# sjtuytc/UnboundedNeRFPytorch

Hardware: NVIDIA B200
Metric: ray-samples/sec (fwd+bwd train step) 8192x512 (higher is better)
Workload: dtype f32

## Files before the change

### include/ubnerf_b200.h

```cpp
#ifndef UBNERF_B200_H_
#define UBNERF_B200_H_

#include <stdint.h>

#ifdef __cplusplus
extern "C" {
#endif
#if defined(__GNUC__)
#pragma GCC visibility push(default)
#endif

#define UBN_ABI_VERSION 3

int ubn_abi_version(void);
const char* ubn_last_error_string(void);
int64_t ubn_launch_count(void);
void ubn_reset_launch_count(void);


int ubn_infer_t_minmax(const float* rays_o, const float* rays_d, const float* xyz_min, const float* xyz_max,
                       float near, float far, int64_t n_rays, float* t_min, float* t_max, void* stream);

int ubn_infer_n_samples(const float* rays_d, const float* t_min, const float* t_max, float stepdist,
                        int64_t n_rays, int64_t* n_samples, void* stream);
// ... 164 lines not shown
                          const UbnGridDesc* k0_desc, const UbnMarchCfg* cfg, int64_t n_rays,
                          const uint8_t* flags, const int64_t* offsets, const float* grad_feat,
                          float* grad_k0, void* stream);

int ubn_march_density_bwd(const float* rays_o, const float* rays_d, const float* t_table,
                          const UbnGridDesc* density_desc, const UbnMarchCfg* cfg, int64_t n_rays,
                          const float* density, const float* alpha, const float* weight, const float* T,
                          const uint8_t* flags, const float* alphainv_last, const int64_t* offsets,
                          const float* g_weight, const float* g_alpha, const float* g_density,
                          const float* g_last, float* grad_density_grid, void* stream);

int ubn_rgbnet_fwd(const float* feat, const float* view_bias, const int64_t* ray_id, const float* W1k, const float* W2,
                   const float* b2, const float* W3, const float* b3, int64_t n_pts, float* rgb, float* h1_save,
                   float* h2_save, void* stream);
int ubn_rgbnet_fwd_tc(const float* feat, const float* view_bias, const int64_t* ray_id, const float* W1k, const float* W2,
                      const float* b2, const float* W3, const float* b3, int64_t n_pts, float* rgb, float* h1_save,
                      float* h2_save, uint32_t* h1_mask, int single_pass, void* stream);
int ubn_rgbnet_bwd(const float* feat, const int64_t* ray_id, const float* W1k, const float* W2, const float* W3,
                   const float* rgb, const float* h1_save, const float* h2_save, const float* grad_rgb, int64_t n_pts,
                   float* grad_feat, float* grad_view_bias, float* grad_W1k, float* grad_W2, float* grad_b2,
                   float* grad_W3, float* grad_b3, void* stream);

int ubn_rgbnet_bwd_tc_data(const float* W2, const float* W3, const float* rgb, const float* h1_save, const float* h2_save,
                           const float* grad_rgb, int64_t n_pts, float* dz1_out, float* grad_W2, void* stream);
int ubn_rgbnet_bwd_small(const float* feat, const int64_t* ray_id, const float* W1k, const float* W3, const float* rgb,
                         const float* h2_save, const float* grad_rgb, const float* dz1, int64_t n_pts, float* grad_feat,
                         float* grad_view_bias, float* grad_W1k, float* grad_b2, float* grad_W3, float* grad_b3, void* stream);

int ubn_rgbnet_bwd_tc_fused(const float* feat, const int64_t* ray_id, const float* W1k, const float* W2, const float* W3,
                            const float* rgb, const float* h1_save, const float* h2_save, const float* grad_rgb, int64_t n_pts,
                            float* grad_feat, float* grad_view_bias, float* grad_W1k, float* grad_W2, float* grad_b2,
                            float* grad_W3, float* grad_b3, uint32_t* h2_mask_scratch, const uint32_t* h1_mask, int single_pass,
                            void* stream);

#if defined(__GNUC__)
#pragma GCC visibility pop
#endif
#ifdef __cplusplus
}
#endif
#endif
```

### unboundednerfpytorch_b200/_cabi.py

```python
import ctypes
import os

import torch

_HERE = os.path.dirname(os.path.abspath(__file__))
LIB_PATH = os.path.join(_HERE, 'libubnerf_b200.so')

c_i64 = ctypes.c_int64
c_i32 = ctypes.c_int32
c_int = ctypes.c_int
c_f = ctypes.c_float
c_p = ctypes.c_void_p


class UbnGridDesc(ctypes.Structure):
    _fields_ = [('P', c_i32), ('C', c_i32), ('X', c_i32), ('Y', c_i32), ('Z', c_i32), ('num_freqs', c_i32),
                ('stride_p', c_i64), ('stride_c', c_i64), ('stride_v', c_i64),
                ('xyz_min', c_f * 3), ('xyz_max', c_f * 3)]


class UbnMarchCfg(ctypes.Structure):
    _fields_ = [('scene_center', c_f * 3), ('scene_radius', c_f * 3),
                ('contract_B', c_f), ('contract_A', c_f),
                ('contracted_norm', c_i32), ('n_samples', c_i32),
                ('act_shift', c_f), ('interval', c_f), ('fast_color_thres', c_f),
                ('use_cumdist', c_i32), ('cumdist_thres', c_f),
                ('use_maskcache', c_i32), ('mask_sz', c_i32 * 3), ('mask_scale', c_f * 3), ('mask_shift', c_f * 3)]


ABI_VERSION = 3
FLAG_QUERIED, FLAG_LISTED, FLAG_SCANNED, FLAG_KEEP, FLAG_INNER = 1, 2, 4, 8, 16

_SIGNATURES = {
    'ubn_abi_version': [],
    'ubn_last_error_string': [],
    'ubn_launch_count': [],
    'ubn_reset_launch_count': [],
    'ubn_infer_t_minmax': [c_p, c_p, c_p, c_p, c_f, c_f, c_i64, c_p, c_p, c_p],
    'ubn_infer_n_samples': [c_p, c_p, c_p, c_f, c_i64, c_p, c_p],
    'ubn_infer_ray_start_dir': [c_p, c_p, c_p, c_i64, c_p, c_p, c_p],
    'ubn_sample_pts_count': [c_p, c_p, c_p, c_p, c_f, c_f, c_f, c_i64, c_p, c_p, c_p, c_p, c_p, c_p],
    'ubn_sample_pts_emit': [c_p, c_p, c_p, c_p, c_p, c_p, c_f, c_i64, c_i64, c_p, c_p, c_p, c_p, c_p],
    'ubn_sample_ndc_pts_on_rays': [c_p, c_p, c_p, c_p, c_i64, c_i64, c_p, c_p, c_p],
    'ubn_sample_bg_pts_on_rays': [c_p, c_p, c_p, c_f, c_i64, c_i64, c_p, c_p],
    'ubn_maskcache_lookup': [c_p, c_p, c_p, c_p, c_i64, c_i64, c_i64, c_i64, c_p, c_p],
    'ubn_raw2alpha': [c_p, c_f, c_f, c_p, c_i64, c_p, c_p, c_p],
    'ubn_raw2alpha_backward': [c_p, c_p, c_f, c_p, c_i64, c_p, c_p],
    'ubn_alpha2weight': [c_p, c_p, c_i64, c_i64, c_p, c_p, c_p, c_p, c_p, c_p],
    'ubn_alpha2weight_backward': [c_p, c_p, c_p, c_p, c_p, c_p, c_i64, c_i64, c_p, c_p, c_p, c_p],
    'ubn_segment_sum': [c_p, c_i64, c_p, c_i64, c_i64, c_p, c_p, c_p, c_p],
    'ubn_rgbnet_fwd': [c_p] * 8 + [c_i64] + [c_p] * 4,
    'ubn_rgbnet_fwd_tc': [c_p] * 8 + [c_i64] + [c_p] * 4 + [c_int, c_p],
    'ubn_rgbnet_bwd_tc_data': [c_p] * 6 + [c_i64] + [c_p] * 3,
    'ubn_rgbnet_bwd_small': [c_p] * 8 + [c_i64] + [c_p] * 7,
    'ubn_rgbnet_bwd': [c_p] * 9 + [c_i64] + [c_p] * 8,
    'ubn_rgbnet_bwd_tc_fused': [c_p] * 9 + [c_i64] + [c_p] * 9 + [c_int, c_p],
    'ubn_total_variation_add_grad': [c_p, c_p, c_f, c_f, c_f, c_i64, c_i64, c_i64, c_i64, c_i64, c_int, c_p],
    'ubn_adam_upd': [c_p, c_p, c_p, c_p, c_p, c_i64, c_int, c_f, c_f, c_f, c_f, c_int, c_p],
    'ubn_tv_adam_fused': [c_p, c_p, c_p, c_p, c_f, c_f, c_f, c_i64, c_i64, c_i64, c_i64, c_i64, c_int, c_int,
                          c_f, c_f, c_f, c_f, c_int, c_int, c_p],
    'ubn_tv_adam_pingpong': [c_p, c_p, c_p, c_p, c_p, c_f, c_f, c_f, c_i64, c_i64, c_i64, c_i64, c_i64, c_int, c_int,
                             c_f, c_f, c_f, c_f, c_int, c_int, c_p],
    'ubn_tv_adam_peer': [c_p, c_p, c_p, c_int, c_p, c_p, c_f, c_f, c_f, c_i64, c_i64, c_i64, c_i64, c_i64, c_int, c_i64, c_i64,
                         c_int, c_f, c_f, c_f, c_f, c_int, c_p],
    'ubn_lattice_alpha': [c_p, ctypes.POINTER(UbnGridDesc), c_p, c_p, c_i64, c_i64, c_i64, c_f, c_f, c_p, c_p],
    'ubn_maxpool3_gt_and': [c_p, c_i64, c_i64, c_i64, c_f, c_p, c_p],
    'ubn_resample_grid': [c_p, ctypes.POINTER(UbnGridDesc), c_p, ctypes.POINTER(UbnGridDesc), c_p],
    'ubn_view_scatter_ones': [c_p, c_p, c_i64, c_i64, c_f, c_f, c_f, ctypes.POINTER(UbnGridDesc), c_p, c_p],
    'ubn_count_gt': [c_p, c_f, c_i64, c_p, c_p],
    'ubn_maskout_near_cam': [c_p, c_i64, c_i64, c_i64, c_i64, c_p, c_i64, c_f, c_f, c_p],
    'ubn_cumdist_thres': [c_p, c_f, c_i64, c_i64, c_p, c_p],
    'ubn_get_rays_of_a_view': [c_int, c_int, c_p, c_p, c_int, c_int, c_int, c_int, c_int, c_int, c_p, c_p, c_p, c_p, c_p],
    'ubn_gather_rays': [c_p, c_p, c_int, c_p, c_i64, c_i64, c_p, c_p],
    'ubn_composite_fwd': [c_p, c_p, c_p, c_i64, c_i64, c_p, c_p, c_p, c_p],
    'ubn_composite_bwd': [c_p, c_p, c_p, c_p, c_i64, c_p, c_p, c_p],
    'ubn_distortion_loss': [c_p, c_p, c_p, c_i64, c_i64, c_f, c_p, c_p, c_p, c_p, c_p, c_i64, c_p],
    'ubn_render_loss': [c_p] * 7 + [c_i64, c_i64] + [c_f] * 6 + [c_p] * 6 + [c_i64, c_p],
    'ubn_grid_sample_fwd': [c_p, ctypes.POINTER(UbnGridDesc), c_p, c_i64, c_p, c_p],
    'ubn_grid_sample_bwd': [c_p, ctypes.POINTER(UbnGridDesc), c_p, c_i64, c_p, c_p],
    'ubn_march_density_fwd': [c_p, c_p, c_p, c_p, ctypes.POINTER(UbnGridDesc), c_p, ctypes.POINTER(UbnMarchCfg), c_i64,
                              c_p, c_p, c_p, c_p, c_p, c_p, c_p, c_p],
    'ubn_exclusive_scan_i32': [c_p, c_i64, c_p, c_p, c_p],
    'ubn_march_feature_fwd': [c_p, c_p, c_p, c_p, ctypes.POINTER(UbnGridDesc), ctypes.POINTER(UbnMarchCfg), c_i64,
                              c_p, c_p, c_p, c_p, c_p, c_p, c_p, c_p, c_p, c_p, c_p, c_p, c_p, c_p],
    'ubn_march_feature_fwd_tma': [c_p, c_p, c_p, c_p, ctypes.POINTER(UbnGridDesc), ctypes.POINTER(UbnMarchCfg), c_i64,
                                  c_p, c_p, c_p, c_p, c_p, c_p, c_p, c_p, c_p, c_p, c_p, c_p, c_p, c_p, c_p],
    'ubn_set_feature_kernel': [c_int],
    'ubn_get_feature_kernel': [],
    'ubn_set_density_scatter': [c_int],
# ... 99 lines not shown
```

### unboundednerfpytorch_b200/csrc/shade_tc.cu

```cuda
#include <algorithm>

#include "common.cuh"

namespace ubn {

namespace tc {

constexpr int kRows = 128;
constexpr int kHidden = 128;
constexpr int kFeat = 12;
constexpr int kK1 = 16;
constexpr uint32_t kPanelBytes = kRows * 16;
constexpr uint32_t kLBO = kPanelBytes;
constexpr uint32_t kSBO = 128;

constexpr uint32_t oW2hi = 0;
constexpr uint32_t oW2lo = oW2hi + (kHidden / 4) * kPanelBytes;
constexpr uint32_t oW1hi = oW2lo + (kHidden / 4) * kPanelBytes;
constexpr uint32_t oW1lo = oW1hi + (kK1 / 4) * kPanelBytes;
constexpr uint32_t oA1hi = oW1lo + (kK1 / 4) * kPanelBytes;
constexpr uint32_t oA1lo = oA1hi + (kK1 / 4) * kPanelBytes;
constexpr uint32_t oW3 = oA1lo + (kK1 / 4) * kPanelBytes;
constexpr uint32_t oB2 = oW3 + 3 * kHidden * 4;
constexpr uint32_t oBar = oB2 + kHidden * 4;
// ... 237 lines not shown
        for (int e = 0; e < 4; ++e) {
          const uint32_t hb = tf32_hi_bits(hs[e]);
          hi[q * 4 + e] = hb;
          lo[q * 4 + e] = __float_as_uint(hs[e] - __uint_as_float(hb));
        }
      }
      tmem_st32(tmem + lane_base + cA2hi + c * 32, hi);
      if (kThreePass) tmem_st32(tmem + lane_base + cA2lo + c * 32, lo);
      tmem_st_wait();
      tc_fence_before();
      __syncthreads();
      if (warp == 0 && elect_one()) {
        tc_fence_after();
#pragma unroll
        for (int hh = 0; hh < kHalves; ++hh) {
#pragma unroll
          for (int k4 = 0; k4 < 4; ++k4) {
            const int ks = (hh * kChunksPerHalf + cc) * 4 + k4;
            mma_ts(tmem + cD2, tmem + cA2hi + ks * 8, dW2hi + ks * kStep, (cc > 0 || hh > 0 || k4 > 0) ? 1u : 0u);
            if (kThreePass) {
              mma_ts(tmem + cD2, tmem + cA2lo + ks * 8, dW2hi + ks * kStep, 1);
              mma_ts(tmem + cD2, tmem + cA2hi + ks * 8, dW2lo + ks * kStep, 1);
            }
          }
        }
        if (cc == kChunksPerHalf - 1) mma_commit(bar_addr);
      }
      if (kSave) {
        if (kPanel && h1_mask) {
          uint32_t w = 0;
#pragma unroll
          for (int e = 31; e >= 0; --e) w = __funnelshift_l(__float_as_uint(__fsub_rn(0.f, v[e])), w, 1);
          h1_mask[tile * 512 + c * 128 + rtid] = live ? w : 0u;
          float* stg = reinterpret_cast<float*>(smem + oStg + warp * kStgBytesPerWarp);
          const int ln = tid & 31;
#pragma unroll
          for (int q = 0; q < 8; ++q)
            *reinterpret_cast<float4*>(stg + ln * kStgStride + q * 4) = make_float4(v[q * 4], v[q * 4 + 1], v[q * 4 + 2], v[q * 4 + 3]);
          __syncwarp();
          float* dstT = h1_out + tile * (kRows * kHidden) + (int64_t)(8 * (warp & 3)) * (kHidden * 4) + (c * 32 + ln) * 4;
#pragma unroll
          for (int q = 0; q < 8; ++q)
            *reinterpret_cast<float4*>(dstT + q * (kHidden * 4)) =
                make_float4(stg[(4 * q) * kStgStride + ln], stg[(4 * q + 1) * kStgStride + ln], stg[(4 * q + 2) * kStgStride + ln],
                            stg[(4 * q + 3) * kStgStride + ln]);
          __syncwarp();
        } else if (kPanel) {
          float4* dst = reinterpret_cast<float4*>(h1_out + tile * (kRows * kHidden) + (int64_t)(c * 8) * (kRows * 4) + rtid * 4);
#pragma unroll
          for (int q = 0; q < 8; ++q) dst[q * kRows] = make_float4(v[q * 4], v[q * 4 + 1], v[q * 4 + 2], v[q * 4 + 3]);
        } else {
          warp_store_chunk(reinterpret_cast<float*>(smem + oStg + warp * kStgBytesPerWarp), v,
                           h1_out + (tile * kRows + (warp & 3) * 32) * kHidden, c * 32, n_pts - (tile * kRows + (warp & 3) * 32), tid & 31);
        }
      }
    }
    mbar_wait(bar_addr, phase);
    phase ^= 1;
    tc_fence_after();
    float p0 = 0.f, p1 = 0.f, p2 = 0.f;
#pragma unroll 1
    for (int cc = 0; cc < kChunksPerHalf; ++cc) {
      const int c = half * kChunksPerHalf + cc;
      float v[32];
      tmem_ld32(tmem + lane_base + cD2 + c * 32, v);
#pragma unroll
      for (int q = 0; q < 8; ++q) {
        const float4 bb = *reinterpret_cast<const float4*>(sB2 + c * 32 + q * 4);
        const float4 wa = *reinterpret_cast<const float4*>(sW3 + c * 32 + q * 4);
        const float4 wb = *reinterpret_cast<const float4*>(sW3 + kHidden + c * 32 + q * 4);
        const float4 wc = *reinterpret_cast<const float4*>(sW3 + 2 * kHidden + c * 32 + q * 4);
        const float h0 = fmaxf(v[q * 4] + bb.x, 0.f), h1v = fmaxf(v[q * 4 + 1] + bb.y, 0.f);
        const float h2v = fmaxf(v[q * 4 + 2] + bb.z, 0.f), h3 = fmaxf(v[q * 4 + 3] + bb.w, 0.f);
        v[q * 4] = h0; v[q * 4 + 1] = h1v; v[q * 4 + 2] = h2v; v[q * 4 + 3] = h3;
        p0 = fmaf(h3, wa.w, fmaf(h2v, wa.z, fmaf(h1v, wa.y, fmaf(h0, wa.x, p0))));
        p1 = fmaf(h3, wb.w, fmaf(h2v, wb.z, fmaf(h1v, wb.y, fmaf(h0, wb.x, p1))));
        p2 = fmaf(h3, wc.w, fmaf(h2v, wc.z, fmaf(h1v, wc.y, fmaf(h0, wc.x, p2))));
      }
      if (kSave) {
// ... 1303 lines not shown
      for (int ks = 0; ks < (int)(kK / 8); ++ks) {
        mma_ss(tmem + cAcc, dAhi + ks * kStepK, dBhi + ks * kStepK, (!fresh || ks > 0) ? 1u : 0u);
        if (kThree) {
          mma_ss(tmem + cAcc, dAlo + ks * kStepK, dBhi + ks * kStepK, 1);
          mma_ss(tmem + cAcc, dAhi + ks * kStepK, dBlo + ks * kStepK, 1);
        }
      }
      mma_commit(bar_addr);
    }
    pending = true;
    prefetch(rd + 1);
  }
  if (pending) {
    mbar_wait(bar_addr, phase);
    tc_fence_after();
    fold(n_folded == 0);
#pragma unroll 1
    for (int c = 0; c < 2; ++c) {
      float v[32];
      tmem_ld32(my_tmem + cSum + c * 32, v);
      float* dst = gW2 + ((warp & 3) * 32 + lane) * kHidden + (warp >> 2) * 64 + c * 32;
#pragma unroll
      for (int e = 0; e < 32; ++e) atomicAdd(dst + e, v[e]);
    }
  }
#pragma unroll
  for (int i = 0; i < 4; ++i) atomicAdd(sB2 + 32 * i + lane, accb[i]);
  tc_fence_before();
  __syncthreads();
  if (tid < kHidden && gb2) atomicAdd(gb2 + tid, sB2[tid]);
  if (warp == 0) asm volatile("tcgen05.dealloc.cta_group::1.sync.aligned.b32 %0, 256;" ::"r"(tmem) : "memory");
}

}
}

using namespace ubn;

extern "C" int ubn_rgbnet_fwd_tc(const float* feat, const float* view_bias, const int64_t* ray_id, const float* W1k,
                                 const float* W2, const float* b2, const float* W3, const float* b3, int64_t n_pts,
                                 float* rgb, float* h1_save, float* h2_save, uint32_t* h1_mask, int single_pass, void* stream) {
  if (n_pts <= 0) return 0;
  const bool save = h1_save != nullptr && h2_save != nullptr;
  const int64_t n_tiles = (n_pts + tc::kRows - 1) / tc::kRows;
  const unsigned grid = (unsigned)std::min<int64_t>(kNumSMs, n_tiles);
  cudaStream_t st = as_stream(stream);
#define UBN_TC_LAUNCH_H(SAVE, THREE, H, P)                                                                                \
  do {                                                                                                                  \
    cudaError_t e = cudaFuncSetAttribute(tc::k_shade_fwd_tc<SAVE, THREE, H, P>, cudaFuncAttributeMaxDynamicSharedMemorySize, \
                                         (int)tc::kSmemBytes);                                                          \
    if (e != cudaSuccess) return finish(e);                                                                             \
    tc::k_shade_fwd_tc<SAVE, THREE, H, P><<<grid, tc::kRows * H, tc::kSmemBytes, st>>>(feat, view_bias, ray_id, W1k, W2, b2, W3, \
                                                                                        b3, n_pts, rgb, h1_save, h2_save,    \
                                                                                        (SAVE && P) ? h1_mask : nullptr);    \
  } while (0)
#define UBN_TC_LAUNCH(SAVE, THREE, P)                                \
  do {                                                               \
    if (four_warps) UBN_TC_LAUNCH_H(SAVE, THREE, 1, P);              \
    else UBN_TC_LAUNCH_H(SAVE, THREE, 2, P);                         \
  } while (0)
  const bool four_warps = (single_pass & 2) != 0, panel = (single_pass & 4) != 0;
  single_pass &= 1;
  if (save && panel) {
    if (single_pass) UBN_TC_LAUNCH(true, false, true); else UBN_TC_LAUNCH(true, true, true);
  } else if (save) {
    if (single_pass) UBN_TC_LAUNCH(true, false, false); else UBN_TC_LAUNCH(true, true, false);
  } else {
    if (single_pass) UBN_TC_LAUNCH(false, false, false); else UBN_TC_LAUNCH(false, true, false);
  }
#undef UBN_TC_LAUNCH
#undef UBN_TC_LAUNCH_H
  UBN_LAUNCH_CHECK();
  return 0;
}


extern "C" int ubn_rgbnet_bwd_tc_data(const float* W2, const float* W3, const float* rgb, const float* h1_save,
                                      const float* h2_save, const float* grad_rgb, int64_t n_pts, float* dz1_out,
                                      float* grad_W2, void* stream) {
  if (n_pts <= 0) return 0;
  cudaStream_t st = as_stream(stream);
  {
    const int64_t n_tiles = (n_pts + tc::kRows - 1) / tc::kRows;
    const unsigned grid = (unsigned)std::min<int64_t>(kNumSMs, n_tiles);
    cudaError_t e = cudaFuncSetAttribute(tc::k_shade_bwd_tc<false>, cudaFuncAttributeMaxDynamicSharedMemorySize,
                                         (int)tc::bw::kSmemBytesB);
    if (e != cudaSuccess) return finish(e);
    tc::k_shade_bwd_tc<false><<<grid, tc::kRows, tc::bw::kSmemBytesB, st>>>(W2, W3, rgb, h1_save, h2_save, grad_rgb, n_pts,
                                                                            dz1_out, grad_W2);
    UBN_LAUNCH_CHECK();
  }
  {
    const int64_t n_rounds = (n_pts + tc::dw::kK - 1) / tc::dw::kK;
    const unsigned grid = (unsigned)std::min<int64_t>((int64_t)kNumSMs * tc::dw::kCtasPerSM, n_rounds);
    cudaError_t e = cudaFuncSetAttribute(tc::k_shade_dw2_tc<true, false>, cudaFuncAttributeMaxDynamicSharedMemorySize,
                                         (int)tc::dw::kSmemBytesD);
    if (e != cudaSuccess) return finish(e);
    tc::k_shade_dw2_tc<true, false><<<grid, tc::dw::kThreadsDW, tc::dw::kSmemBytesD, st>>>(W3, rgb, h1_save, h2_save, grad_rgb, n_pts,
                                                                                   grad_W2);
    UBN_LAUNCH_CHECK();
  }
  return 0;
}


extern "C" int ubn_rgbnet_bwd_tc_fused(const float* feat, const int64_t* ray_id, const float* W1k, const float* W2, const float* W3,
                                       const float* rgb, const float* h1_save, const float* h2_save, const float* grad_rgb,
                                       int64_t n_pts, float* grad_feat, float* grad_view_bias, float* grad_W1k, float* grad_W2,
                                       float* grad_b2, float* grad_W3, float* grad_b3, uint32_t* h2_mask_scratch,
                                       const uint32_t* h1_mask, int single_pass, void* stream) {
  if (n_pts <= 0) return 0;
  cudaStream_t st = as_stream(stream);
  {
    const int64_t n_tiles = (n_pts + tc::kRows - 1) / tc::kRows;
    const unsigned grid = (unsigned)std::min<int64_t>(kNumSMs, n_tiles);
#define UBN_BF(T)                                                                                                              \
    do {                                                                                                                       \
      cudaError_t e = cudaFuncSetAttribute(tc::k_shade_bwd_fused<T>, cudaFuncAttributeMaxDynamicSharedMemorySize,              \
                                           (int)tc::bf::kSmemBytesF);                                                          \
      if (e != cudaSuccess) return finish(e);                                                                                  \
      tc::k_shade_bwd_fused<T><<<grid, tc::kRows, tc::bf::kSmemBytesF, st>>>(feat, ray_id, W1k, W2, W3, rgb, h1_save, h2_save, grad_rgb, \
                                                                             n_pts, grad_feat, grad_view_bias, grad_W1k, grad_b2,       \
                                                                             grad_W3, grad_b3);                                         \
    } while (0)
#define UBN_BFW(T, P, M1)                                                                                                      \
    do {                                                                                                                       \
      cudaError_t e = cudaFuncSetAttribute(tc::k_shade_bwd_fused_ws<T, P, M1>, cudaFuncAttributeMaxDynamicSharedMemorySize,    \
                                           (int)tc::bf2::kSmemBytesF2);                                                        \
      if (e != cudaSuccess) return finish(e);                                                                                  \
      tc::k_shade_bwd_fused_ws<T, P, M1><<<grid, 2 * tc::kRows, tc::bf2::kSmemBytesF2, st>>>(                                  \
          feat, ray_id, W1k, W2, W3, rgb, h1_save, h2_save, grad_rgb, n_pts, grad_feat, grad_view_bias, grad_W1k, grad_b2, grad_W3,   \
          grad_b3, (P) ? h2_mask_scratch : nullptr, h1_mask);                                                                  \
    } while (0)
    const bool one_pass = (single_pass & 1) != 0, plain = (single_pass & 2) != 0, panel = (single_pass & 4) != 0;
    if (plain && panel) return finish(cudaErrorInvalidValue);
    if (plain)      { if (one_pass) UBN_BF(false); else UBN_BF(true); }
    else if (panel && h1_mask && h2_mask_scratch) { if (one_pass) UBN_BFW(false, true, true); else UBN_BFW(true, true, true); }
    else if (panel)            { if (one_pass) UBN_BFW(false, true, false); else UBN_BFW(true, true, false); }
    else                       { if (one_pass) UBN_BFW(false, false, false); else UBN_BFW(true, false, false); }
#undef UBN_BFW
#undef UBN_BF
    UBN_LAUNCH_CHECK();
  }
  {
    const int64_t n_rounds = (n_pts + tc::dw::kK - 1) / tc::dw::kK;
    const unsigned grid = (unsigned)std::min<int64_t>((int64_t)kNumSMs * tc::dw::kCtasPerSM, n_rounds);
#define UBN_DW(T, P)                                                                                                           \
    do {                                                                                                                       \
      cudaError_t e = cudaFuncSetAttribute(tc::k_shade_dw2_tc<T, P>, cudaFuncAttributeMaxDynamicSharedMemorySize,              \
                                           (int)tc::dw::kSmemBytesD);                                                          \
      if (e != cudaSuccess) return finish(e);                                                                                  \
      tc::k_shade_dw2_tc<T, P><<<grid, tc::dw::kThreadsDW, tc::dw::kSmemBytesD, st>>>(W3, rgb, h1_save, h2_save, grad_rgb, n_pts, grad_W2); \
    } while (0)
#define UBN_DWM(T)                                                                                                             \
    do {                                                                                                                       \
      cudaError_t e = cudaFuncSetAttribute(tc::k_shade_dw2_mask_tc<T>, cudaFuncAttributeMaxDynamicSharedMemorySize,            \
                                           (int)tc::dw::kSmemBytesD);                                                          \
      if (e != cudaSuccess) return finish(e);                                                                                  \
      tc::k_shade_dw2_mask_tc<T><<<grid, tc::dw::kThreadsDW, tc::dw::kSmemBytesD, st>>>(W3, rgb, h1_save, h2_mask_scratch, grad_rgb, n_pts, \
                                                                                      grad_W2, grad_b2);                       \
    } while (0)
    const bool from_masks = (single_pass & 4) && !(single_pass & 2) && h2_mask_scratch != nullptr && h1_mask != nullptr;
    if (from_masks)           { if (single_pass & 1) UBN_DWM(false); else UBN_DWM(true); }
    else if (single_pass & 4) { if (single_pass & 1) UBN_DW(false, true); else UBN_DW(true, true); }
    else                      { if (single_pass & 1) UBN_DW(false, false); else UBN_DW(true, false); }
#undef UBN_DWM
#undef UBN_DW
    UBN_LAUNCH_CHECK();
  }
  return 0;
}
```

### unboundednerfpytorch_b200/shade.py

```python
import torch

import os

from . import _cabi, ops
from ._cabi import c_i64, c_int, check, ptr, stream_of

MODE = os.environ.get('UBN_RGBNET_MODE', 'tc3')
BWD_MODE = os.environ.get('UBN_RGBNET_BWD_MODE', 'fused')
USE_MASKS = os.environ.get('UBN_RGBNET_MASKS', '1') == '1'


class _ShadeFn(torch.autograd.Function):
    @staticmethod
    def forward(ctx, feat, vb, ray_id, W1k, W2, b2, W3, b3, need_grad):
        feat, vb, ray_id = feat.contiguous(), vb.contiguous(), ray_id.contiguous()
        W1k, W2, b2, W3, b3 = (t.contiguous() for t in (W1k, W2, b2, W3, b3))
        M = feat.shape[0]
        dev = feat.device
        rgb = torch.empty(M, 3, dtype=torch.float32, device=dev)
        need_grad = bool(need_grad) and any(ctx.needs_input_grad)
        panel = need_grad and MODE in ('tc3', 'tc1', 'tc3w4') and BWD_MODE == 'fused'
        rows = -(-M // 128) * 128 if panel else M
        h1 = torch.empty(rows, 128, dtype=torch.float32, device=dev) if need_grad else None
        h2 = torch.empty(rows, 128, dtype=torch.float32, device=dev) if need_grad else None
        m1 = torch.empty(rows * 4, dtype=torch.int32, device=dev) if (panel and USE_MASKS) else None
        with ops._Guard(feat) as lib:
            with _cabi.timed('rgbnet_fwd'):
                if MODE in ('tc3', 'tc1', 'tc3w4'):
                    check(lib.ubn_rgbnet_fwd_tc(ptr(feat), ptr(vb), ptr(ray_id), ptr(W1k), ptr(W2), ptr(b2), ptr(W3), ptr(b3),
                                                c_i64(M), ptr(rgb), ptr(h1), ptr(h2), ptr(m1),
                                                c_int((1 if MODE == 'tc1' else 0) | (2 if MODE == 'tc3w4' else 0) | (4 if panel else 0)),
                                                stream_of(feat)))
                else:
                    check(lib.ubn_rgbnet_fwd(ptr(feat), ptr(vb), ptr(ray_id), ptr(W1k), ptr(W2), ptr(b2), ptr(W3), ptr(b3),
                                             c_i64(M), ptr(rgb), ptr(h1), ptr(h2), stream_of(feat)))
        if need_grad:
            ctx.save_for_backward(feat, ray_id, W1k, W2, W3, rgb, h1, h2)
            ctx.m1 = m1
            ctx.n_rays = vb.shape[0]
            ctx.panel = panel
            ctx.bwd_mode = BWD_MODE
        return rgb

    @staticmethod
    @torch.autograd.function.once_differentiable
    def backward(ctx, g_rgb):
        feat, ray_id, W1k, W2, W3, rgb, h1, h2 = ctx.saved_tensors
        dev = feat.device
        M = feat.shape[0]
        g_rgb = g_rgb.contiguous()
        g_feat = torch.empty_like(feat)
        z = lambda *s: torch.zeros(*s, dtype=torch.float32, device=dev)
        g_vb, gW1k, gW2, gb2, gW3, gb3 = z(ctx.n_rays, 128), z(128, 12), z(128, 128), z(128), z(3, 128), z(3)
        with ops._Guard(feat) as lib:
            bwd_mode = ctx.bwd_mode
            if bwd_mode in ('fused', 'fused4'):
                masks = torch.empty(-(-M // 128) * 512, dtype=torch.int32, device=dev) if (ctx.panel and ctx.m1 is not None) else None
                with _cabi.timed('rgbnet_bwd'):
                    check(lib.ubn_rgbnet_bwd_tc_fused(ptr(feat), ptr(ray_id), ptr(W1k), ptr(W2), ptr(W3), ptr(rgb), ptr(h1), ptr(h2),
                                                      ptr(g_rgb), c_i64(M), ptr(g_feat), ptr(g_vb), ptr(gW1k), ptr(gW2), ptr(gb2),
                                                      ptr(gW3), ptr(gb3), ptr(masks), ptr(ctx.m1 if bwd_mode == 'fused' else None), c_int((1 if MODE == 'tc1' else 0) | (2 if bwd_mode == 'fused4' else 0) | (4 if ctx.panel else 0)),
                                                      stream_of(feat)))
                return g_feat, g_vb, None, gW1k, gW2, gb2, gW3, gb3, None
            if bwd_mode == 'tc3':
                dz1 = torch.empty(M, 128, dtype=torch.float32, device=dev)
                with _cabi.timed('rgbnet_bwd'):
                    check(lib.ubn_rgbnet_bwd_tc_data(ptr(W2), ptr(W3), ptr(rgb), ptr(h1), ptr(h2), ptr(g_rgb), c_i64(M),
                                                     ptr(dz1), ptr(gW2), stream_of(feat)))
                with _cabi.timed('rgbnet_bwd_small'):
                    check(lib.ubn_rgbnet_bwd_small(ptr(feat), ptr(ray_id), ptr(W1k), ptr(W3), ptr(rgb), ptr(h2), ptr(g_rgb),
                                                   ptr(dz1), c_i64(M), ptr(g_feat), ptr(g_vb), ptr(gW1k), ptr(gb2), ptr(gW3),
                                                   ptr(gb3), stream_of(feat)))
                return g_feat, g_vb, None, gW1k, gW2, gb2, gW3, gb3, None
            with _cabi.timed('rgbnet_bwd'):
                check(lib.ubn_rgbnet_bwd(ptr(feat), ptr(ray_id), ptr(W1k), ptr(W2), ptr(W3), ptr(rgb), ptr(h1), ptr(h2),
                                         ptr(g_rgb), c_i64(M), ptr(g_feat), ptr(g_vb), ptr(gW1k), ptr(gW2), ptr(gb2),
                                         ptr(gW3), ptr(gb3), stream_of(feat)))
        return g_feat, g_vb, None, gW1k, gW2, gb2, gW3, gb3, None


def supported(rgbnet, k0_dim):
    try:
        l1, l2, l3 = rgbnet[0], rgbnet[2][0], rgbnet[3]
    except Exception:
        return False
    return (len(rgbnet) == 4 and k0_dim == 12 and l1.weight.shape[0] == 128 and tuple(l2.weight.shape) == (128, 128)
            and tuple(l3.weight.shape) == (3, 128) and l1.weight.is_cuda and l1.weight.dtype == torch.float32)


def shade(rgbnet, k0, view_emb, ray_id):
    l1, l2, l3 = rgbnet[0], rgbnet[2][0], rgbnet[3]
# ... 4 lines not shown
```

Before: 337.1 million.

## Recompute h1 activations in backward instead of saving them in forward

The forward pass no longer writes the full h1 activation tensor when masks are in use. A new backward kernel recomputes h1 on tensor cores from feat, W1k and the saved view bias, then accumulates grad_W2 and grad_b2 from it. This removes an M×128 float write in forward and the matching read in backward, at the cost of extra layer-1 MMA work and per-row gathers of the view bias in backward.

Result: slower. 325.4 million, median of 6 (-3.4%).

```diff
diff --git a/include/ubnerf_b200.h b/include/ubnerf_b200.h
--- a/include/ubnerf_b200.h
+++ b/include/ubnerf_b200.h
@@ -220,6 +220,11 @@
                             float* grad_feat, float* grad_view_bias, float* grad_W1k, float* grad_W2, float* grad_b2,
                             float* grad_W3, float* grad_b3, uint32_t* h2_mask_scratch, const uint32_t* h1_mask, int single_pass,
                             void* stream);
+int ubn_rgbnet_bwd_tc_recompute(const float* feat, const float* view_bias, const int64_t* ray_id, const float* W1k,
+                                const float* W2, const float* W3, const float* rgb, const float* h2_save, const float* grad_rgb,
+                                int64_t n_pts, float* grad_feat, float* grad_view_bias, float* grad_W1k, float* grad_W2,
+                                float* grad_b2, float* grad_W3, float* grad_b3, uint32_t* h2_mask_scratch,
+                                const uint32_t* h1_mask, int single_pass, void* stream);
 
 #if defined(__GNUC__)
 #pragma GCC visibility pop
diff --git a/unboundednerfpytorch_b200/_cabi.py b/unboundednerfpytorch_b200/_cabi.py
--- a/unboundednerfpytorch_b200/_cabi.py
+++ b/unboundednerfpytorch_b200/_cabi.py
@@ -55,6 +55,7 @@
     'ubn_rgbnet_bwd_small': [c_p] * 8 + [c_i64] + [c_p] * 7,
     'ubn_rgbnet_bwd': [c_p] * 9 + [c_i64] + [c_p] * 8,
     'ubn_rgbnet_bwd_tc_fused': [c_p] * 9 + [c_i64] + [c_p] * 9 + [c_int, c_p],
+    'ubn_rgbnet_bwd_tc_recompute': [c_p] * 9 + [c_i64] + [c_p] * 9 + [c_int, c_p],
     'ubn_total_variation_add_grad': [c_p, c_p, c_f, c_f, c_f, c_i64, c_i64, c_i64, c_i64, c_i64, c_int, c_p],
     'ubn_adam_upd': [c_p, c_p, c_p, c_p, c_p, c_i64, c_int, c_f, c_f, c_f, c_f, c_int, c_p],
     'ubn_tv_adam_fused': [c_p, c_p, c_p, c_p, c_f, c_f, c_f, c_i64, c_i64, c_i64, c_i64, c_i64, c_int, c_int,
diff --git a/unboundednerfpytorch_b200/csrc/shade_tc.cu b/unboundednerfpytorch_b200/csrc/shade_tc.cu
--- a/unboundednerfpytorch_b200/csrc/shade_tc.cu
+++ b/unboundednerfpytorch_b200/csrc/shade_tc.cu
@@ -293,19 +293,21 @@
 #pragma unroll
           for (int e = 31; e >= 0; --e) w = __funnelshift_l(__float_as_uint(__fsub_rn(0.f, v[e])), w, 1);
           h1_mask[tile * 512 + c * 128 + rtid] = live ? w : 0u;
-          float* stg = reinterpret_cast<float*>(smem + oStg + warp * kStgBytesPerWarp);
-          const int ln = tid & 31;
-#pragma unroll
-          for (int q = 0; q < 8; ++q)
-            *reinterpret_cast<float4*>(stg + ln * kStgStride + q * 4) = make_float4(v[q * 4], v[q * 4 + 1], v[q * 4 + 2], v[q * 4 + 3]);
-          __syncwarp();
-          float* dstT = h1_out + tile * (kRows * kHidden) + (int64_t)(8 * (warp & 3)) * (kHidden * 4) + (c * 32 + ln) * 4;
-#pragma unroll
-          for (int q = 0; q < 8; ++q)
-            *reinterpret_cast<float4*>(dstT + q * (kHidden * 4)) =
-                make_float4(stg[(4 * q) * kStgStride + ln], stg[(4 * q + 1) * kStgStride + ln], stg[(4 * q + 2) * kStgStride + ln],
-                            stg[(4 * q + 3) * kStgStride + ln]);
-          __syncwarp();
+          if (h1_out != nullptr) {
+            float* stg = reinterpret_cast<float*>(smem + oStg + warp * kStgBytesPerWarp);
+            const int ln = tid & 31;
+#pragma unroll
+            for (int q = 0; q < 8; ++q)
+              *reinterpret_cast<float4*>(stg + ln * kStgStride + q * 4) = make_float4(v[q * 4], v[q * 4 + 1], v[q * 4 + 2], v[q * 4 + 3]);
+            __syncwarp();
+            float* dstT = h1_out + tile * (kRows * kHidden) + (int64_t)(8 * (warp & 3)) * (kHidden * 4) + (c * 32 + ln) * 4;
+#pragma unroll
+            for (int q = 0; q < 8; ++q)
+              *reinterpret_cast<float4*>(dstT + q * (kHidden * 4)) =
+                  make_float4(stg[(4 * q) * kStgStride + ln], stg[(4 * q + 1) * kStgStride + ln], stg[(4 * q + 2) * kStgStride + ln],
+                              stg[(4 * q + 3) * kStgStride + ln]);
+            __syncwarp();
+          }
         } else if (kPanel) {
           float4* dst = reinterpret_cast<float4*>(h1_out + tile * (kRows * kHidden) + (int64_t)(c * 8) * (kRows * 4) + rtid * 4);
 #pragma unroll
@@ -1675,6 +1677,315 @@
   if (warp == 0) asm volatile("tcgen05.dealloc.cta_group::1.sync.aligned.b32 %0, 256;" ::"r"(tmem) : "memory");
 }
 
+namespace dr {
+constexpr int kThreadsDR = 256;
+constexpr uint32_t kOpBytes = (dw::kK / 4) * kPanelBytes;
+constexpr uint32_t oV1hi = 0;
+constexpr uint32_t oV1lo = oV1hi + (kK1 / 4) * kPanelBytes;
+constexpr uint32_t oXhi = oV1lo + (kK1 / 4) * kPanelBytes;
+constexpr uint32_t oXlo = oXhi + (kK1 / 4) * kPanelBytes;
+constexpr uint32_t oZ = oXlo + (kK1 / 4) * kPanelBytes;
+constexpr uint32_t oRayR = oZ + 4 * kOpBytes;
+constexpr uint32_t oB2R = oRayR + kRows * 8;
+constexpr uint32_t oBarR = oB2R + kHidden * 4;
+constexpr uint32_t kSmemBytesR = oBarR + 32;
+constexpr uint32_t cAcc = 0, cSum = 128, cH1 = 256;
+constexpr uint32_t kHalfCols = 128;
+constexpr uint32_t kIdescN64 = (1u << 4) | (2u << 7) | (2u << 10) | ((uint32_t)(64 >> 3) << 17) | ((uint32_t)(kRows >> 4) << 24);
+__device__ __forceinline__ void mma_ss_n64(uint32_t d_tmem, uint64_t a_desc, uint64_t b_desc, uint32_t accumulate) {
+  asm volatile(
+      "{\n\t.reg .pred p;\n\tsetp.ne.b32 p, %4, 0;\n\t"
+      "tcgen05.mma.cta_group::1.kind::tf32 [%0], %1, %2, %3, p;\n\t}\n" ::"r"(d_tmem),
+      "l"(a_desc), "l"(b_desc), "r"(kIdescN64), "r"(accumulate)
+      : "memory");
+}
+}
+
+template <bool kThree>
+__global__ void __launch_bounds__(dr::kThreadsDR, 1) k_shade_dw2_h1r_tc(
+    const float* __restrict__ feat, const float* __restrict__ vb, const int64_t* __restrict__ ray_id, const float* __restrict__ W1k,
+    const float* __restrict__ W3, const float* __restrict__ rgb, const uint32_t* __restrict__ h2_mask, const float* __restrict__ g_rgb,
+    int64_t n_pts, float* __restrict__ gW2, float* __restrict__ gb2) {
+  using namespace dr;
+  constexpr int kFlushR = dw::kFlush;
+  extern __shared__ __align__(1024) uint8_t smem[];
+  const int tid = threadIdx.x, warp = tid >> 5, lane = tid & 31;
+  uint64_t* bar = reinterpret_cast<uint64_t*>(smem + oBarR);
+  uint32_t* tmem_slot = reinterpret_cast<uint32_t*>(smem + oBarR + 24);
+  int64_t* sRay = reinterpret_cast<int64_t*>(smem + oRayR);
+  float* sB2 = reinterpret_cast<float*>(smem + oB2R);
+  const uint32_t bar_l1 = smem_u32(bar), bar_buf0 = smem_u32(bar + 1);
+
+  stage_weights(W1k, kFeat, kK1, smem + oV1hi, smem + oV1lo, tid, kThreadsDR);
+  if (tid < kHidden) sB2[tid] = 0.f;
+  if (tid == 0) {
+    for (int b = 0; b < 3; ++b) mbar_init(smem_u32(bar + b), 1);
+    asm volatile("fence.mbarrier_init.release.cluster;" ::: "memory");
+  }
+  if (warp == 0) {
+    asm volatile("tcgen05.alloc.cta_group::1.sync.aligned.shared::cta.b32 [%0], 512;" ::"r"(smem_u32(tmem_slot)) : "memory");
+    asm volatile("tcgen05.relinquish_alloc_permit.cta_group::1.sync.aligned;" ::: "memory");
+  }
+  fence_async_smem();
+  tc_fence_before();
+  __syncthreads();
+  tc_fence_after();
+  const uint32_t tmem = *tmem_slot;
+  constexpr uint64_t kStepK = (uint64_t)((2 * kPanelBytes) >> 4);
+  const uint64_t dW1hi = make_desc(smem_u32(smem + oV1hi)), dW1lo = make_desc(smem_u32(smem + oV1lo));
+  const uint64_t dXhi = make_desc(smem_u32(smem + oXhi)), dXlo = make_desc(smem_u32(smem + oXlo));
+  const uint64_t dZhi0 = make_desc(smem_u32(smem + oZ)), dZlo0 = make_desc(smem_u32(smem + oZ + kOpBytes));
+  constexpr uint64_t kBufStep = (uint64_t)((2 * kOpBytes) >> 4);
+
+  const int64_t n_tiles = (n_pts + kRows - 1) / kRows;
+  const int64_t t_per_cta = (n_tiles + gridDim.x - 1) / gridDim.x;
+  const int64_t t_begin = (int64_t)blockIdx.x * t_per_cta, t_end = min(n_tiles, t_begin + t_per_cta);
+  const uint32_t lane_base = (uint32_t)((warp & 3) * 32) << 16;
+  const uint32_t my_tmem = tmem + lane_base + (uint32_t)(warp >> 2) * 64;
+  const int k_unit = (warp & 3) * 32 + lane;
+
+  float w3a[4], w3b[4], w3c[4];
+#pragma unroll
+  for (int i = 0; i < 4; ++i) {
+    w3a[i] = W3[32 * i + lane]; w3b[i] = W3[kHidden + 32 * i + lane]; w3c[i] = W3[2 * kHidden + 32 * i + lane];
+  }
+  const uint32_t row_off = (uint32_t)warp * kPanelBytes + (uint32_t)lane * 16;
+  float accb[4] = {0.f, 0.f, 0.f, 0.f};
+  uint4 pm[4];
+  float4 po[3], pg[3];
+  auto prefetch = [&](int64_t rd) {
+    const bool on = rd < t_end * kFlushR;
+    const int64_t tile = rd >> 2;
+    const int r_in = (int)(rd & 3) * 32 + warp * 4;
+    const int64_t row0 = rd * dw::kK + warp * 4;
+#pragma unroll
+    for (int i = 0; i < 4; ++i) {
+      pm[i] = make_uint4(0, 0, 0, 0);
+      if (on) pm[i] = __ldg(reinterpret_cast<const uint4*>(h2_mask + tile * 512 + i * 128 + r_in));
+    }
+    if (on && row0 + 4 <= n_pts) {
+      const float4* o = reinterpret_cast<const float4*>(rgb + row0 * 3);
+      const float4* g = reinterpret_cast<const float4*>(g_rgb + row0 * 3);
+      po[0] = __ldg(o); po[1] = __ldg(o + 1); po[2] = __ldg(o + 2);
+      pg[0] = __ldg(g); pg[1] = __ldg(g + 1); pg[2] = __ldg(g + 2);
+    } else {
+      float fo[12], fg[12];
+#pragma unroll
+      for (int e = 0; e < 12; ++e) {
+        const bool ok = on && row0 * 3 + e < n_pts * 3;
+        fo[e] = ok ? rgb[row0 * 3 + e] : 0.f;
+        fg[e] = ok ? g_rgb[row0 * 3 + e] : 0.f;
+      }
+      po[0] = make_float4(fo[0], fo[1], fo[2], fo[3]); po[1] = make_float4(fo[4], fo[5], fo[6], fo[7]); po[2] = make_float4(fo[8], fo[9], fo[10], fo[11]);
+      pg[0] = make_float4(fg[0], fg[1], fg[2], fg[3]); pg[1] = make_float4(fg[4], fg[5], fg[6], fg[7]); pg[2] = make_float4(fg[8], fg[9], fg[10], fg[11]);
+    }
+  };
+  auto stage_dz2 = [&](int64_t rd, int b) {
+    float d0[4], d1[4], d2[4];
+    {
+      const float fo[12] = {po[0].x, po[0].y, po[0].z, po[0].w, po[1].x, po[1].y, po[1].z, po[1].w, po[2].x, po[2].y, po[2].z, po[2].w};
+      const float fg[12] = {pg[0].x, pg[0].y, pg[0].z, pg[0].w, pg[1].x, pg[1].y, pg[1].z, pg[1].w, pg[2].x, pg[2].y, pg[2].z, pg[2].w};
+#pragma unroll
+      for (int t = 0; t < 4; ++t) {
+        d0[t] = fg[3 * t] * (fo[3 * t] * (1.f - fo[3 * t]));
+        d1[t] = fg[3 * t + 1] * (fo[3 * t + 1] * (1.f - fo[3 * t + 1]));
+        d2[t] = fg[3 * t + 2] * (fo[3 * t + 2] * (1.f - fo[3 * t + 2]));
+      }
+    }
+    uint8_t* buf = smem + oZ + (uint32_t)b * 2 * kOpBytes;
+#pragma unroll
+    for (int i = 0; i < 4; ++i) {
+      const uint32_t mw[4] = {pm[i].x, pm[i].y, pm[i].z, pm[i].w};
+      uint4 zh;
+      float4 zl;
+      uint32_t* zhp = &zh.x; float* zlp = &zl.x;
+#pragma unroll
+      for (int t = 0; t < 4; ++t) {
+        const float z = ((mw[t] >> lane) & 1u) ? fmaf(d2[t], w3c[i], fmaf(d1[t], w3b[i], d0[t] * w3a[i])) : 0.f;
+        accb[i] += z;
+        zhp[t] = tf32_hi_bits(z);
+        zlp[t] = z - __uint_as_float(zhp[t]);
+      }
+      const uint32_t off = row_off + (uint32_t)i * 512;
+      *reinterpret_cast<uint4*>(buf + off) = zh;
+      *reinterpret_cast<float4*>(buf + kOpBytes + off) = zl;
+    }
+    prefetch(rd + 1);
+  };
+  auto fold = [&](bool first) {
+#pragma unroll 1
+    for (int c = 0; c < 4; ++c) {
+      float v[16], sum[16];
+      tmem_ld16(my_tmem + cAcc + c * 16, v);
+      if (!first) {
+        tmem_ld16(my_tmem + cSum + c * 16, sum);
+#pragma unroll
+        for (int e = 0; e < 16; ++e) v[e] = __fadd_rn(sum[e], v[e]);
+      }
+      tmem_st16(my_tmem + cSum + c * 16, v);
+    }
+    tmem_st_wait();
+  };
+  float4 xr[3];
+  int64_t rayr = 0;
+  auto fetch_x = [&](int64_t t) {
+    const int64_t r = t * kRows + tid;
+    const bool ok = tid < kRows && t < t_end && r < n_pts;
+#pragma unroll
+    for (int p = 0; p < 3; ++p) xr[p] = ok ? __ldg(reinterpret_cast<const float4*>(feat + r * kFeat + p * 4)) : make_float4(0, 0, 0, 0);
+    rayr = ok ? ray_id[r] : 0;
+  };
+
+  uint32_t ph_l1 = 0, ph_buf = 0, busy = 0;
+  auto wait_buf = [&](int b) {
+    if ((busy >> b) & 1u) {
+      mbar_wait(bar_buf0 + 8 * b, (ph_buf >> b) & 1u);
+      ph_buf ^= 1u << b;
+      busy &= ~(1u << b);
+    }
+  };
+  auto sync_for_mma = [&]() {
+    fence_async_smem();
+    tc_fence_before();
+    __syncthreads();
+  };
+  auto mma_round = [&](int r, int b) {
+#pragma unroll
+    for (int ks = 0; ks < (int)(dw::kK / 8); ++ks) {
+      const uint32_t a = tmem + cH1 + (uint32_t)(r >> 1) * kHalfCols + (uint32_t)((r & 1) * 32 + ks * 8);
+      const uint64_t zh = dZhi0 + b * kBufStep + ks * kStepK, zl = dZlo0 + b * kBufStep + ks * kStepK;
+      mma_ts(tmem + cAcc, a, zh, (r > 0 || ks > 0) ? 1u : 0u);
+      if (kThree) {
+        mma_ts(tmem + cAcc, a, zl, 1);
+        mma_ts(tmem + cAcc, a + 64, zh, 1);
+      }
+    }
+    mma_commit(bar_buf0 + 8 * b);
+  };
+  auto mma_layer1 = [&](int h) {
+    const uint64_t xo = (uint64_t)((h * 64 * 16) >> 4);
+#pragma unroll
+    for (int ks = 0; ks < kK1 / 8; ++ks) {
+      mma_ss_n64(tmem + cH1 + h * kHalfCols, dW1hi + ks * kStepK, dXhi + xo + ks * kStepK, ks > 0);
+      if (kThree) {
+        mma_ss_n64(tmem + cH1 + h * kHalfCols, dW1hi + ks * kStepK, dXlo + xo + ks * kStepK, 1);
+        mma_ss_n64(tmem + cH1 + h * kHalfCols, dW1lo + ks * kStepK, dXhi + xo + ks * kStepK, 1);
+      }
+    }
+    mma_commit(bar_l1);
+  };
+  auto epilogue_h1 = [&](int64_t tile, int h) {
+    mbar_wait(bar_l1, ph_l1);
+    ph_l1 ^= 1;
+    tc_fence_after();
+    const int s0 = h * 64 + (warp >> 2) * 32;
+    const uint32_t col = cH1 + (uint32_t)h * kHalfCols + (uint32_t)(warp >> 2) * 32;
+    float v[32];
+    tmem_ld32(tmem + lane_base + col, v);
+    uint32_t hi[32], lo[32];
+#pragma unroll
+    for (int e = 0; e < 32; ++e) {
+      const float b = __ldg(vb + sRay[s0 + e] * kHidden + k_unit);
+      const float hv = (tile * kRows + s0 + e < n_pts) ? fmaxf(v[e] + b, 0.f) : 0.f;
+      hi[e] = tf32_hi_bits(hv);
+      lo[e] = __float_as_uint(hv - __uint_as_float(hi[e]));
+    }
+    tmem_st32(tmem + lane_base + col, hi);
+    if (kThree) tmem_st32(tmem + lane_base + col + 64, lo);
+    tmem_st_wait();
+  };
+  auto stage_x = [&]() {
+    if (tid < kRows) {
+#pragma unroll
+      for (int p = 0; p < 4; ++p) {
+        const float4 v = p < 3 ? xr[p] : make_float4(0, 0, 0, 0);
+        uint4 hi;
+        float4 lo;
+        hi.x = tf32_hi_bits(v.x); hi.y = tf32_hi_bits(v.y); hi.z = tf32_hi_bits(v.z); hi.w = tf32_hi_bits(v.w);
+        lo.x = v.x - __uint_as_float(hi.x); lo.y = v.y - __uint_as_float(hi.y);
+        lo.z = v.z - __uint_as_float(hi.z); lo.w = v.w - __uint_as_float(hi.w);
+        *reinterpret_cast<uint4*>(smem + oXhi + p * kPanelBytes + tid * 16) = hi;
+        *reinterpret_cast<float4*>(smem + oXlo + p * kPanelBytes + tid * 16) = lo;
+      }
+      sRay[tid] = rayr;
+    }
+  };
+
+  fetch_x(t_begin);
+  if (t_begin < t_end) {
+    prefetch(t_begin * kFlushR);
+    stage_x();
+    sync_for_mma();
+    if (warp == 0 && elect_one()) { tc_fence_after(); mma_layer1(0); }
+    fetch_x(t_begin + 1);
+    epilogue_h1(t_begin, 0);
+  }
+  int n_folded = 0;
+  for (int64_t tile = t_begin; tile < t_end; ++tile) {
+    const int64_t rd0 = tile * kFlushR;
+    wait_buf(0);
+    stage_dz2(rd0, 0);
+    wait_buf(1);
+    if (tile > t_begin) {
+      tc_fence_after();
+      fold(n_folded == 0);
+      ++n_folded;
+    }
+    sync_for_mma();
+    if (warp == 0 && elect_one()) {
+      tc_fence_after();
+      mma_round(0, 0);
+      mma_layer1(1);
+    }
+    busy |= 1u;
+    stage_dz2(rd0 + 1, 1);
+    sync_for_mma();
+    if (warp == 0 && elect_one()) { tc_fence_after(); mma_round(1, 1); }
+    busy |= 2u;
+    epilogue_h1(tile, 1);
+    wait_buf(0);
+    stage_dz2(rd0 + 2, 0);
+    sync_for_mma();
+    if (warp == 0 && elect_one()) { tc_fence_after(); mma_round(2, 0); }
+    busy |= 1u;
+    const bool more = tile + 1 < t_end;
+    if (more) {
+      stage_x();
+      fetch_x(tile + 2);
+    }
+    wait_buf(1);
+    stage_dz2(rd0 + 3, 1);
+    sync_for_mma();
+    if (warp == 0 && elect_one()) {
+      tc_fence_after();
+      mma_round(3, 1);
+      if (more) mma_layer1(0);
+    }
+    busy |= 2u;
+    if (more) epilogue_h1(tile + 1, 0);
+  }
+  if (t_begin < t_end) {
+    wait_buf(0);
+    wait_buf(1);
+    tc_fence_after();
+    fold(n_folded == 0);
+#pragma unroll 1
+    for (int c = 0; c < 2; ++c) {
+      float v[32];
+      tmem_ld32(my_tmem + cSum + c * 32, v);
+      float* dst = gW2 + (int64_t)((warp >> 2) * 64 + c * 32) * kHidden + k_unit;
+#pragma unroll
+      for (int e = 0; e < 32; ++e) atomicAdd(dst + e * kHidden, v[e]);
+    }
+  }
+#pragma unroll
+  for (int i = 0; i < 4; ++i) atomicAdd(sB2 + 32 * i + lane, accb[i]);
+  tc_fence_before();
+  __syncthreads();
+  if (tid < kHidden && gb2) atomicAdd(gb2 + tid, sB2[tid]);
+  if (warp == 0) asm volatile("tcgen05.dealloc.cta_group::1.sync.aligned.b32 %0, 512;" ::"r"(tmem) : "memory");
+}
+
 }
 }
 
@@ -1684,7 +1995,8 @@
                                  const float* W2, const float* b2, const float* W3, const float* b3, int64_t n_pts,
                                  float* rgb, float* h1_save, float* h2_save, uint32_t* h1_mask, int single_pass, void* stream) {
   if (n_pts <= 0) return 0;
-  const bool save = h1_save != nullptr && h2_save != nullptr;
+  const bool panel = (single_pass & 4) != 0;
+  const bool save = h2_save != nullptr && (h1_save != nullptr || (panel && h1_mask != nullptr));
   const int64_t n_tiles = (n_pts + tc::kRows - 1) / tc::kRows;
   const unsigned grid = (unsigned)std::min<int64_t>(kNumSMs, n_tiles);
   cudaStream_t st = as_stream(stream);
@@ -1702,7 +2014,7 @@
     if (four_warps) UBN_TC_LAUNCH_H(SAVE, THREE, 1, P);              \
     else UBN_TC_LAUNCH_H(SAVE, THREE, 2, P);                         \
   } while (0)
-  const bool four_warps = (single_pass & 2) != 0, panel = (single_pass & 4) != 0;
+  const bool four_warps = (single_pass & 2) != 0;
   single_pass &= 1;
   if (save && panel) {
     if (single_pass) UBN_TC_LAUNCH(true, false, true); else UBN_TC_LAUNCH(true, true, true);
@@ -1747,13 +2059,10 @@
 }
 
 
-extern "C" int ubn_rgbnet_bwd_tc_fused(const float* feat, const int64_t* ray_id, const float* W1k, const float* W2, const float* W3,
-                                       const float* rgb, const float* h1_save, const float* h2_save, const float* grad_rgb,
-                                       int64_t n_pts, float* grad_feat, float* grad_view_bias, float* grad_W1k, float* grad_W2,
-                                       float* grad_b2, float* grad_W3, float* grad_b3, uint32_t* h2_mask_scratch,
-                                       const uint32_t* h1_mask, int single_pass, void* stream) {
-  if (n_pts <= 0) return 0;
-  cudaStream_t st = as_stream(stream);
+static int bwd_fused_launch1(const float* feat, const int64_t* ray_id, const float* W1k, const float* W2, const float* W3,
+                             const float* rgb, const float* h1_save, const float* h2_save, const float* grad_rgb, int64_t n_pts,
+                             float* grad_feat, float* grad_view_bias, float* grad_W1k, float* grad_b2, float* grad_W3,
+                             float* grad_b3, uint32_t* h2_mask_scratch, const uint32_t* h1_mask, int single_pass, cudaStream_t st) {
   {
     const int64_t n_tiles = (n_pts + tc::kRows - 1) / tc::kRows;
     const unsigned grid = (unsigned)std::min<int64_t>(kNumSMs, n_tiles);
@@ -1785,6 +2094,22 @@
 #undef UBN_BF
     UBN_LAUNCH_CHECK();
   }
+  return 0;
+}
+
+
+extern "C" int ubn_rgbnet_bwd_tc_fused(const float* feat, const int64_t* ray_id, const float* W1k, const float* W2, const float* W3,
+                                       const float* rgb, const float* h1_save, const float* h2_save, const float* grad_rgb,
+                                       int64_t n_pts, float* grad_feat, float* grad_view_bias, float* grad_W1k, float* grad_W2,
+                                       float* grad_b2, float* grad_W3, float* grad_b3, uint32_t* h2_mask_scratch,
+                                       const uint32_t* h1_mask, int single_pass, void* stream) {
+  if (n_pts <= 0) return 0;
+  cudaStream_t st = as_stream(stream);
+  {
+    const int rc = bwd_fused_launch1(feat, ray_id, W1k, W2, W3, rgb, h1_save, h2_save, grad_rgb, n_pts, grad_feat, grad_view_bias,
+                                     grad_W1k, grad_b2, grad_W3, grad_b3, h2_mask_scratch, h1_mask, single_pass, st);
+    if (rc) return rc;
+  }
   {
     const int64_t n_rounds = (n_pts + tc::dw::kK - 1) / tc::dw::kK;
     const unsigned grid = (unsigned)std::min<int64_t>((int64_t)kNumSMs * tc::dw::kCtasPerSM, n_rounds);
@@ -1813,3 +2138,32 @@
   }
   return 0;
 }
+
+
+extern "C" int ubn_rgbnet_bwd_tc_recompute(const float* feat, const float* view_bias, const int64_t* ray_id, const float* W1k,
+                                           const float* W2, const float* W3, const float* rgb, const float* h2_save,
+                                           const float* grad_rgb, int64_t n_pts, float* grad_feat, float* grad_view_bias,
+                                           float* grad_W1k, float* grad_W2, float* grad_b2, float* grad_W3, float* grad_b3,
+                                           uint32_t* h2_mask_scratch, const uint32_t* h1_mask, int single_pass, void* stream) {
+  if (n_pts <= 0) return 0;
+  if (!view_bias || !h2_mask_scratch || !h1_mask || (single_pass & 2)) return finish(cudaErrorInvalidValue);
+  cudaStream_t st = as_stream(stream);
+  const int rc = bwd_fused_launch1(feat, ray_id, W1k, W2, W3, rgb, nullptr, h2_save, grad_rgb, n_pts, grad_feat, grad_view_bias,
+                                   grad_W1k, grad_b2, grad_W3, grad_b3, h2_mask_scratch, h1_mask, (single_pass & 1) | 4, st);
+  if (rc) return rc;
+  const int64_t n_tiles = (n_pts + tc::kRows - 1) / tc::kRows;
+  const unsigned grid = (unsigned)std::min<int64_t>(kNumSMs, n_tiles);
+#define UBN_DWR(T)                                                                                                             \
+  do {                                                                                                                         \
+    cudaError_t e = cudaFuncSetAttribute(tc::k_shade_dw2_h1r_tc<T>, cudaFuncAttributeMaxDynamicSharedMemorySize,              \
+                                         (int)tc::dr::kSmemBytesR);                                                            \
+    if (e != cudaSuccess) return finish(e);                                                                                    \
+    tc::k_shade_dw2_h1r_tc<T><<<grid, tc::dr::kThreadsDR, tc::dr::kSmemBytesR, st>>>(feat, view_bias, ray_id, W1k, W3, rgb,    \
+                                                                                     h2_mask_scratch, grad_rgb, n_pts, grad_W2, \
+                                                                                     grad_b2);                                 \
+  } while (0)
+  if (single_pass & 1) UBN_DWR(false); else UBN_DWR(true);
+#undef UBN_DWR
+  UBN_LAUNCH_CHECK();
+  return 0;
+}
diff --git a/unboundednerfpytorch_b200/shade.py b/unboundednerfpytorch_b200/shade.py
--- a/unboundednerfpytorch_b200/shade.py
+++ b/unboundednerfpytorch_b200/shade.py
@@ -21,9 +21,10 @@
         need_grad = bool(need_grad) and any(ctx.needs_input_grad)
         panel = need_grad and MODE in ('tc3', 'tc1', 'tc3w4') and BWD_MODE == 'fused'
         rows = -(-M // 128) * 128 if panel else M
-        h1 = torch.empty(rows, 128, dtype=torch.float32, device=dev) if need_grad else None
+        recompute = panel and USE_MASKS
+        h1 = torch.empty(rows, 128, dtype=torch.float32, device=dev) if (need_grad and not recompute) else None
         h2 = torch.empty(rows, 128, dtype=torch.float32, device=dev) if need_grad else None
-        m1 = torch.empty(rows * 4, dtype=torch.int32, device=dev) if (panel and USE_MASKS) else None
+        m1 = torch.empty(rows * 4, dtype=torch.int32, device=dev) if recompute else None
         with ops._Guard(feat) as lib:
             with _cabi.timed('rgbnet_fwd'):
                 if MODE in ('tc3', 'tc1', 'tc3w4'):
@@ -35,7 +36,7 @@
                     check(lib.ubn_rgbnet_fwd(ptr(feat), ptr(vb), ptr(ray_id), ptr(W1k), ptr(W2), ptr(b2), ptr(W3), ptr(b3),
                                              c_i64(M), ptr(rgb), ptr(h1), ptr(h2), stream_of(feat)))
         if need_grad:
-            ctx.save_for_backward(feat, ray_id, W1k, W2, W3, rgb, h1, h2)
+            ctx.save_for_backward(feat, ray_id, W1k, W2, W3, rgb, h1, h2, vb if recompute else None)
             ctx.m1 = m1
             ctx.n_rays = vb.shape[0]
             ctx.panel = panel
@@ -45,7 +46,7 @@
     @staticmethod
     @torch.autograd.function.once_differentiable
     def backward(ctx, g_rgb):
-        feat, ray_id, W1k, W2, W3, rgb, h1, h2 = ctx.saved_tensors
+        feat, ray_id, W1k, W2, W3, rgb, h1, h2, vb = ctx.saved_tensors
         dev = feat.device
         M = feat.shape[0]
         g_rgb = g_rgb.contiguous()
@@ -57,6 +58,12 @@
             if bwd_mode in ('fused', 'fused4'):
                 masks = torch.empty(-(-M // 128) * 512, dtype=torch.int32, device=dev) if (ctx.panel and ctx.m1 is not None) else None
                 with _cabi.timed('rgbnet_bwd'):
+                    if vb is not None:
+                        check(lib.ubn_rgbnet_bwd_tc_recompute(ptr(feat), ptr(vb), ptr(ray_id), ptr(W1k), ptr(W2), ptr(W3), ptr(rgb),
+                                                              ptr(h2), ptr(g_rgb), c_i64(M), ptr(g_feat), ptr(g_vb), ptr(gW1k),
+                                                              ptr(gW2), ptr(gb2), ptr(gW3), ptr(gb3), ptr(masks), ptr(ctx.m1),
+                                                              c_int(1 if MODE == 'tc1' else 0), stream_of(feat)))
+                        return g_feat, g_vb, None, gW1k, gW2, gb2, gW3, gb3, None
                     check(lib.ubn_rgbnet_bwd_tc_fused(ptr(feat), ptr(ray_id), ptr(W1k), ptr(W2), ptr(W3), ptr(rgb), ptr(h1), ptr(h2),
                                                       ptr(g_rgb), c_i64(M), ptr(g_feat), ptr(g_vb), ptr(gW1k), ptr(gW2), ptr(gb2),
                                                       ptr(gW3), ptr(gb3), ptr(masks), ptr(ctx.m1 if bwd_mode == 'fused' else None), c_int((1 if MODE == 'tc1' else 0) | (2 if bwd_mode == 'fused4' else 0) | (4 if ctx.panel else 0)),
```
